# BruceCanovas/supersurfel_fusion

Measured on AMD Instinct MI355X. Metric: frames_per_sec, higher is better.
Workload: dtype f32; 1 GPU; 640x480 synthetic RGB-D orbit (seed 1234), map seeded with 1000000 supersurfels (~993223 live, ~86081 visible), reference rgbd_benchmark parameters, extract+ICP+fuse per frame; width=640, height=480, n_model=993223, n_visible=86081, superpixels=1200, icp_iter_max=10, icp_forced=False, seed_order=seeded, exchange=none, pipeline_depth=2, extract_batch=8

## Files before the change

### supersurfel_fusion_amd/csrc/lab/host_probes.inc

```

int ssf_dbg_last_icp_record(ssf_handle* h, int64_t* out29) {
    if (!h || !out29) return SSF_ERR_INVALID_ARG;
    for (int i = 0; i < 29; i++) out29[i] = h->h_icp_local[i];
    return SSF_OK;
}
int ssf_dbg_device_icp_records(ssf_handle* h, int64_t* out64) {
    if (!h || !out64) return SSF_ERR_INVALID_ARG;
    HCK(hipStreamSynchronize(h->stream));
    HCK(hipMemcpy(out64, h->d_icp, 64 * sizeof(int64_t), hipMemcpyDeviceToHost));
    return SSF_OK;
}
void ssf_dbg_stall_before_match_us(ssf_handle* h, long long us) { if (h) h->dbg_stall_before_match_us = us; }
long long ssf_dbg_assoc_replica_frames(ssf_handle* h) { return h ? h->n_assoc_replica_frames : -1; }
int ssf_dbg_host_times(ssf_handle* h, double* out8) {
    if (!h || !out8) return SSF_ERR_INVALID_ARG;
    for (int i = 0; i < 8; i++) { out8[i] = h->host_us[i]; h->host_us[i] = 0; }
    return SSF_OK;
}
double ssf_dbg_extract_only(ssf_handle* h, const void* const* rgb, const void* const* depth, int nlist, int n) {
    if (!h || !rgb || !depth || nlist <= 0 || !h->pending.empty()) return -1.0;
    int nsub = 0;
    double t0 = 0;
    for (int i = 0; i < n; i++) {
        if (i == n / 4) { for (auto& c : h->ctx) (void)hipStreamSynchronize(c.stream); (void)hipStreamSynchronize(h->stream); t0 = now_us(); }
// ... 46 lines not shown
    (void)hipStreamSynchronize(h->stream);
    float ms = 0.f; (void)hipEventElapsedTime(&ms, e0, e1);
    (void)hipEventDestroy(e0); (void)hipEventDestroy(e1);
    if (blocks2) {
        const int nb = (span + 255) / 256;
        std::vector<uint32_t> bc((size_t)std::max(nb, 1));
        if (nb > 0) (void)hipMemcpy(bc.data(), h->d_bc_oov, (size_t)nb * 4, hipMemcpyDeviceToHost);
        blocks2[0] = nb; blocks2[1] = 0;
        for (int i = 0; i < nb; i++) blocks2[1] += bc[i] != 0u;
    }
    return reps > 0 ? 1000.0 * ms / reps : 0.0;
}
int ssf_dbg_trace_fuse(ssf_handle* h, unsigned long long* out, int cap_wgs, int* arms4, int mode ) {
    if (!h || !h->have_frame || !h->cc || !out || !arms4) return -1;
    arms4[0] = (mode & 2) ? 0 : (h->S + 31) / 32; arms4[1] = (mode & 2) ? 0 : (h->S + 255) / 256; arms4[2] = (mode & 4) ? 0 : (h->n_visible + 255) / 256;
    long long b2[2];
    unsigned long long* d = nullptr;
    const size_t words = (size_t)3 * 65536;
    if (hipMalloc((void**)&d, words * 8) != hipSuccess) return -2;
    (void)hipMemset(d, 0, words * 8);
    set_fuse_trace(d);
    (void)ssf_dbg_time_fuse(h, 1, mode, b2);
    set_fuse_trace(nullptr);
    std::vector<unsigned long long> all(words);
    (void)hipMemcpy(all.data(), d, words * 8, hipMemcpyDeviceToHost);
    (void)hipFree(d);
    int n = 0;
    for (int i = 0; i < 65536; i++) if (all[3 * (size_t)i]) n = i + 1;
    arms4[3] = n - arms4[0] - arms4[1] - arms4[2];
    const int m = n < cap_wgs ? n : cap_wgs;
    std::memcpy(out, all.data(), (size_t)m * 24);
    return m;
}
int ssf_dbg_pass_stats_enable(int on) { set_pass_stats(on ? 1 : 0); return SSF_OK; }
int ssf_dbg_pass_stats(ssf_handle* h, uint32_t* out64) {
    if (!h || !h->active.ctx || !out64) return SSF_ERR_INVALID_ARG;
    HCK(hipStreamSynchronize(h->active.ctx->stream));
    HCK(hipMemcpy(out64, h->active.maps.epoch, 64 * sizeof(uint32_t), hipMemcpyDeviceToHost));
    return SSF_OK;
}
double ssf_dbg_time_pass(ssf_handle* h, int reps, int rgbd, int dbg, int nb) {
    if (!h || !h->active.ctx) return -1.0;
    ExtractCtx& c = *h->active.ctx;
    nb = std::max(1, std::min(nb, h->batch));
    hipEvent_t e0, e1; (void)hipEventCreate(&e0); (void)hipEventCreate(&e1);
    const int ox[4] = {0, 1, 0, 1}, oy[4] = {0, 1, 1, 0};
    for (int i = 0; i < 4; i++) launch_update_pass(h->stream, h->seg, c.maps, nb, 20 + i, ox[i & 3], oy[i & 3], rgbd != 0, dbg);
    (void)hipEventRecord(e0, h->stream);
    for (int i = 0; i < reps; i++) launch_update_pass(h->stream, h->seg, c.maps, nb, 24 + i, ox[i & 3], oy[i & 3], rgbd != 0, dbg);
    (void)hipEventRecord(e1, h->stream);
    (void)hipStreamSynchronize(h->stream);
    float ms = 0.f; (void)hipEventElapsedTime(&ms, e0, e1);
    (void)hipEventDestroy(e0); (void)hipEventDestroy(e1);
    return 1000.0 * ms / reps;
}
int ssf_dbg_trace_pass(ssf_handle* h, int rgbd, int nb, unsigned long long* out, int cap_wgs, int* grid3) {
    if (!h || !h->active.ctx || !out || !grid3) return -1;
    ExtractCtx& c = *h->active.ctx;
    nb = std::max(1, std::min(nb, h->batch));
    const int ox[4] = {0, 1, 0, 1}, oy[4] = {0, 1, 1, 0};
    grid3[0] = (h->cfg.width + 30 + 31) / 32; grid3[1] = (h->cfg.height + 31) / 32; grid3[2] = nb;
    const int n = grid3[0] * grid3[1] * grid3[2];
    unsigned long long* d = nullptr;
    if (hipMalloc((void**)&d, (size_t)n * 40) != hipSuccess) return -2;
    (void)hipMemset(d, 0, (size_t)n * 40);
    for (int i = 0; i < 4; i++) launch_update_pass(h->stream, h->seg, c.maps, nb, 20 + i, ox[i & 3], oy[i & 3], rgbd != 0, 0);
// ... 11 lines not shown
```

### supersurfel_fusion_amd/csrc/ssf_device.hpp

```cpp
#pragma once
#include <hip/hip_runtime.h>
#include <stdint.h>
#include <cstddef>
#include "ssf_math.hpp"
#include "ssf_mailbox.hpp"
#include "ssf_tile_geometry.hpp"
#include "../../include/ssf.h"
#include "../../include/ssf_input.h"
#include "../../include/ssf_dynamic.h"

#ifdef SSF_EXPERIMENTS
#include <stdlib.h>
static inline int ssf_env_int_(const char* name, int dflt) { const char* e = getenv(name); return e ? atoi(e) : dflt; }
#define SSF_ENV_INT(name, dflt) ssf_env_int_("SSF_" name, dflt)
#define SSF_ENV_SET(name) (getenv("SSF_" name) != nullptr)
#define SSF_ENV_STR(name) getenv("SSF_" name)
#define SSF_PROBE(dbg, bits) ((((dbg)) & (bits)) != 0)
#else
#define SSF_PROBE(dbg, bits) (false)
#define SSF_ENV_INT(name, dflt) (dflt)
#define SSF_ENV_SET(name) (false)
#define SSF_ENV_STR(name) ((const char*)nullptr)
#endif

// ... 152 lines not shown
SSF_HD int assoc_stride(int S) { return (S + 15) & ~15; }
SSF_HD size_t assoc_table_words(int S) { return (size_t)(1 + SSF_ASSOC_REPLICAS) * (size_t)assoc_stride(S); }
struct MatchArgs { float zmin, zmax; long long id_offset; unsigned long long* best; uint8_t* matched; int32_t* cand; int rstride; };
struct ClassifyArgs { Cam cam; const float* plane_depth; int delta_t; float conf_thresh, zmin, zmax; int assoc_rstride; };
struct ShardArgs { int rank, nranks, migrate; float tile; };
struct AssocTables { const unsigned long long* best; const uint8_t* matched; const int32_t* cand; int S; int rstride; };
int icp_variant_mode();
void launch_icp(hipStream_t st, const Cam& cam, SurfelSoA model, int n_visible, const uint2* pix2, const float4* fpack,
                Rt T, long long* replicas, unsigned int* ticket,
                long long* sums29, Mailbox* mb, unsigned long long seq, int dbg = -1, IcpGo* go = nullptr,
                unsigned long long go_seq = 0, const struct P2PView* pv = nullptr, int by_tile = 0, const MatchArgs* match = nullptr);
int icp_resident_max_wgs();
void launch_icp_resident(hipStream_t st, const Cam& cam, SurfelSoA model, int n_visible, const uint2* pix2, const float4* fpack, const Rt* T0,
                         long long* replicas, long long* sums29, Mailbox* mb, unsigned long long seq0, IcpGo* go, unsigned int go_base,
                         int last_idx, const MatchArgs* match);
void launch_bin_rows(hipStream_t st, const Cam& cam, SurfelSoA model, int n, Rt T, uint32_t* count, uint32_t* cursor, SurfelSoA out);
size_t bin_buffer_words(const Cam& cam, size_t capacity);
void launch_match(hipStream_t st, const Cam& cam, SurfelSoA model, int n_visible, const uint2* pix2, const float4* fpack,
                  Rt pose, float zmin, float zmax, long long id_offset,
                  unsigned long long* best, uint8_t* matched, int32_t* cand , int S,
                  const int32_t* orig = nullptr );
struct OovStore { SurfelSoA rows; uint8_t* live; int cap; };
#define PART_GROUP 16
#define PART_REPLICAS 8
struct PartitionWs { uint32_t* sup_vis; uint32_t* sup_oov; uint32_t* tot; uint32_t* ticket; uint32_t* other; int words; };
void launch_fuse(hipStream_t st, SurfelSoA model , SurfelSoA frame, Rt pose, int stamp, long long id_offset,
                 int n_visible, const AssocTables& at, int do_update, int capacity, const ShardArgs& sh, Counters* cnt, OovStore oov,
                 int span_upper, const ClassifyArgs& ca, uint8_t* state_vis, uint8_t* state_oov, uint32_t* bc_oov, const PartitionWs& ws,
                 int tail_in_move = 0 );
#ifdef SSF_EXPERIMENTS
void set_pass_stats(int on);
void set_pass_trace(unsigned long long* device_words );
void set_fuse_trace(unsigned long long* device_words );
#endif
struct MoveTotals { int from_tot, nv , head_old, tail_old ; };
void launch_pack_emigrants(hipStream_t st, SurfelSoA model, const AssocTables& at, long long id_offset, int n_visible,
                           const uint8_t* state_vis, int do_update, const ShardArgs& sh, int32_t* table);
void launch_migrate_in(hipStream_t st, SurfelSoA model, const int32_t* table, int S, int capacity, Counters* cnt, const ShardArgs& sh,
                       const ClassifyArgs& ca, Rt pose, int stamp, uint8_t* state_vis, const PartitionWs& ws);
void launch_rehome_split(hipStream_t st, SurfelSoA dense, int n, int n_visible, int rank, int nranks, float tile, uint32_t* bc, int* tot3,
                         SurfelSoA stay, int32_t* table, int table_rows);
void launch_rehome_unpack(hipStream_t st, const int32_t* table, int n, SurfelSoA dst, int base);
void launch_first_frame(hipStream_t st, SurfelSoA model, SurfelSoA frame, Rt pose, int S, int capacity, const ShardArgs& sh, Counters* cnt);
struct NextIcp {
    Cam cam; const uint2* pix2; const float4* fpack;
    Rt T;
    long long* replicas; unsigned int* ticket; long long* sums; Mailbox* mb; unsigned long long seq;
};
void launch_move_rows(hipStream_t st, SurfelSoA vis_src, SurfelSoA vis_dst, OovStore oov, int nv_upper, int span_upper,
                      const uint8_t* state_vis, const uint8_t* state_oov, const uint32_t* bc_oov, const PartitionWs& ws,
                      Counters* cnt , Mailbox* mb, unsigned long long cnt_seq, const NextIcp* next,
                      const struct P2PView* next_pv = nullptr, const MoveTotals* totals = nullptr);
void launch_oov_compact(hipStream_t st, OovStore src, OovStore dst, int span_upper, int new_head, uint32_t* bc_oov, Counters* cnt,
                        int set_span);
struct ModelView { SurfelSoA vis; OovStore oov; int n_visible, nbv, nvs, oov_head, oov_tail, nbo, nslots; };
void launch_align(hipStream_t st, const Cam& cam, const float* spos, const float* slab, const float* snrm, const float* sconf,
                  int n, SurfelSoA frame, const int32_t* label, const float* plane_depth, Rt T, long long* out40);
void launch_fern_codes(hipStream_t st, const uint8_t* rgb, const float* depth, int W, int H, const uint32_t* fpos,
                       const uint8_t* frgb, const float* fdepth, int n, uint8_t* codes);
#define SSF_P2P_MAX_RANKS 8
struct P2PView { unsigned char* peer[SSF_P2P_MAX_RANKS]; int me, nranks, S; unsigned long long seq, timeout_ticks; };
enum { P2P_FLAG_ASSOC = 0, P2P_FLAG_MIGR = 1 };
#define SSF_P2P_HEADER 8192
SSF_HD size_t p2p_slot(int par, int src) { return (size_t)(par * SSF_P2P_MAX_RANKS + src); }
SSF_HD size_t p2p_spad(int S) { return ((size_t)S + 63) & ~(size_t)63; }
SSF_HD size_t p2p_off_icp(int par, int src) { return p2p_slot(par, src) * 320; }
// ... 32 lines not shown
```

### supersurfel_fusion_amd/csrc/ssf_track_fuse.hip

```cpp
#include <stdlib.h>
#include <algorithm>
#include "ssf_rows.hpp"

namespace ssf {

#ifndef ICP_SLOTS
#define ICP_SLOTS 16
#endif
template <bool UNIFORM, typename Emit>
__device__ __forceinline__ void icp_row_terms_(const Cam& cam, const uint2* __restrict__ pix2, const float4* __restrict__ fpack,
                                               const M3& R, const V3& t, const V3& mpos, const V3& mlab, const V3& mnrm, int dbg, Emit emit,
                                               bool live = true) {
    const V3 ps = add(m3_mulv(R, mpos), t);
    if (SSF_PROBE(dbg, 1)) { if (ps.z > 1e30f) emit(28, 1ll); return; }
    const int u = pixel_round(ps.x * cam.fx / ps.z + cam.cx);
    const int v = pixel_round(ps.y * cam.fy / ps.z + cam.cy);
    bool ok = live && u >= 0 && u < cam.W && v >= 0 && v < cam.H;
    if (!UNIFORM && !ok) return;
    size_t q = ok ? (size_t)v * cam.W + u : 0;
    if (SSF_PROBE(dbg, 16)) q = (blockIdx.x * blockDim.x + threadIdx.x) & 0x7ffffu;
    const uint2 pl = pix2[q];
    const int tid = SSF_PROBE(dbg, 8) ? (int)(q & 1023) : (int)pl.x;
    const float zt = __uint_as_float(pl.y);
    float4 f0 = fpack[4 * tid], f1 = fpack[4 * tid + 1];
    asm volatile("" : "+v"(f0.y), "+v"(f1.x));
    ok = ok && (f0.x > 0.0f && zt >= 0.2f && zt <= 5.0f);
    if (!UNIFORM && !ok) return;
    const float dist_color = len3(sub(mlab, v3(f0.y, f0.z, f0.w)));
    const V3 pt = v3(zt * ((float)u - cam.cx) / cam.fx, zt * ((float)v - cam.cy) / cam.fy, zt);
    const V3 nt = v3(f1.x, f1.y, f1.z);
    const V3 ns = unit3(m3_mulv(R, mnrm));
    ok = ok && (dist_color < 20.0f && len3(sub(ps, pt)) < 0.1f && fabsf(dot3(nt, ns)) > 0.8f);
    if (!UNIFORM && !ok) return;
    const V3 d = sub(pt, ps), c1 = cross3(pt, ns), c2 = cross3(ps, nt);
    const float dn1 = dot3(d, ns), dn2 = dot3(d, nt);
    const float x1[6] = {c1.x, c1.y, c1.z, ns.x, ns.y, ns.z};
    const float x2[6] = {c2.x, c2.y, c2.z, nt.x, nt.y, nt.z};
    if (SSF_PROBE(dbg, 2)) { if (x1[0] * x2[0] > 1e30f) emit(0, 1ll); return; }
    const float m10 = (UNIFORM && !ok) ? 0.0f : 1024.0f, m14 = (UNIFORM && !ok) ? 0.0f : 16384.0f;
    float X1[6], X2[6];
#pragma unroll
    for (int i = 0; i < 6; i++) { X1[i] = UNIFORM && !ok ? 0.0f : x1[i] * m10; X2[i] = UNIFORM && !ok ? 0.0f : x2[i] * m10; }
    const float D1 = UNIFORM && !ok ? 0.0f : dn1 * m14, D2 = UNIFORM && !ok ? 0.0f : dn2 * m14;
    int k = 0;
#pragma unroll
    for (int i = 0; i < 6; i++)
#pragma unroll
        for (int j = i; j < 6; j++, k++) emit(k, (long long)fx32r(X1[i] * X1[j] + X2[i] * X2[j]));
#pragma unroll
    for (int i = 0; i < 6; i++) emit(21 + i, (long long)fx32r(D1 * X1[i] + D2 * X2[i]));
    emit(27, fx64((double)(UNIFORM && !ok ? 0.0f : dn2 * dn2), 17592186044416.0, 4611686018427387904.0));
    emit(28, (UNIFORM && !ok) ? 0ll : 1ll);
}
template <typename Emit>
__device__ __forceinline__ void icp_row_terms(const Cam& cam, const uint2* __restrict__ pix2, const float4* __restrict__ fpack,
                                              const M3& R, const V3& t, const V3& mpos, const V3& mlab, const V3& mnrm, int dbg, Emit emit) {
    icp_row_terms_<false>(cam, pix2, fpack, R, t, mpos, mlab, mnrm, dbg, emit);
}
__device__ __forceinline__ void icp_row(const Cam& cam, const uint2* __restrict__ pix2, const float4* __restrict__ fpack,
                                        const M3& R, const V3& t, const V3& mpos, const V3& mlab, const V3& mnrm,
                                        unsigned long long* red, int slot, int dbg) {
    icp_row_terms(cam, pix2, fpack, R, t, mpos, mlab, mnrm, dbg, [&](int k, long long v) { atomicAdd(&red[k * ICP_SLOTS + slot], (unsigned long long)v); });
}
__device__ __forceinline__ void icp_fold(unsigned long long* red, long long* __restrict__ replicas) {
    if (threadIdx.x < 29) {
        unsigned long long tot = 0;
#pragma unroll
        for (int sidx = 0; sidx < ICP_SLOTS; sidx++) tot += red[threadIdx.x * ICP_SLOTS + sidx];
        long long* rep = replicas + (size_t)(blockIdx.x % SSF_ICP_REPLICAS) * 32;
        if (tot != 0) atomic_add_done(reinterpret_cast<unsigned long long*>(&rep[threadIdx.x]), tot);
    }
    asm volatile("s_waitcnt vmcnt(0)" ::: "memory");
    __syncthreads();
}
template <bool P2P>
__device__ __forceinline__ void icp_publish(long long* __restrict__ replicas, long long* __restrict__ sums, Mailbox* mb,
                                            unsigned long long seq, const P2PView& pv, unsigned long long p2p_seq) {
    __shared__ long long part[8 * 32];
    const int field = threadIdx.x & 31, group = threadIdx.x >> 5;
    long long v = 0;
#pragma unroll
    for (int j = 0; j < (SSF_ICP_REPLICAS + 7) / 8; j++) {
        const int r = group + 8 * j;
        if (r < SSF_ICP_REPLICAS) {
            v += __hip_atomic_load(&replicas[r * 32 + field], __ATOMIC_RELAXED, __HIP_MEMORY_SCOPE_AGENT);
// ... 123 lines not shown
                                            float zmax, long long id_offset, unsigned long long* __restrict__ best,
                                            uint8_t* __restrict__ matched, bool wave_agg);
__device__ __forceinline__ void match_sorted_rows(const Cam& cam, const SurfelSoA& sorted, int n_visible, const uint2* __restrict__ pix2,
                                                  const float4* __restrict__ fpack, const Rt& pose, const MatchArgs& ma) {
    for (int j = (int)(xcd_block(blockIdx.x, gridDim.x) * blockDim.x + threadIdx.x); j < n_visible; j += gridDim.x * blockDim.x) {
        const float4* __restrict__ rec = reinterpret_cast<const float4*>(sorted.pos) + 3 * (size_t)j;
        float4 a = rec[0], b = rec[1], c = rec[2];
        asm volatile("" : "+v"(a.x), "+v"(b.x), "+v"(c.x));
        const int oid = __float_as_int(b.w);
        ma.cand[oid] = match_values(cam, a.w, v3(a.x, a.y, a.z), v3(c.x, c.y, c.z), v3(b.x, b.y, b.z), oid, pix2, fpack, pose, ma.zmin, ma.zmax, ma.id_offset, ma.best, ma.matched, true);
    }
}
__device__ __forceinline__ unsigned long long* assoc_bid_table(const MatchArgs& ma) {
    const unsigned int xcc = __builtin_amdgcn_s_getreg((3 << 11) | (0 << 6) | 20) & 7u;
    return ma.rstride ? ma.best + (size_t)(1u + xcc) * (size_t)ma.rstride : ma.best;
}
__device__ __forceinline__ unsigned long long assoc_best(const unsigned long long* __restrict__ best, int f, int rstride) {
    unsigned long long v = best[f];
    if (rstride) {
        unsigned long long r[SSF_ASSOC_REPLICAS];
#pragma unroll
        for (int x = 0; x < SSF_ASSOC_REPLICAS; x++) r[x] = best[(size_t)(1 + x) * (size_t)rstride + f];
#pragma unroll
        for (int x = 0; x < SSF_ASSOC_REPLICAS; x++) v = r[x] < v ? r[x] : v;
    }
    return v;
}
#define SSF_ICP_DBG_COUNTED 0x40000000
#ifndef SSF_ICP_GO_WAIT_TICKS
#define SSF_ICP_GO_WAIT_TICKS 25000000ull
#endif
#ifndef SSF_ICP_NUM_SGPR
#define SSF_ICP_NUM_SGPR 80
#endif
__device__ __forceinline__ int icp_wait_word(IcpGo* go, unsigned int want, unsigned int& w) {
    int ok = 0, told = 0;
    const unsigned int l = threadIdx.x;
    const unsigned int* gw = reinterpret_cast<const unsigned int*>(go);
    const unsigned int weight = icp_go_word_weight(l);
    w = 0u;
    const unsigned long long t0 = wall_clock64();
    for (unsigned int spin = 0; spin < (1u << 24); spin++) {
        w = l < 16u ? __hip_atomic_load(&gw[l], __ATOMIC_RELAXED, __HIP_MEMORY_SCOPE_SYSTEM) : 0u;
        const unsigned int flo = (unsigned int)__builtin_amdgcn_readlane((int)w, 12), fhi = (unsigned int)__builtin_amdgcn_readlane((int)w, 13);
        if (flo == want) {
            if (fhi & 0x80000000u) {
                if ((fhi & SSF_ICP_GO_CHECK_MASK) == icp_go_abort_check(want)) { told = 1; break; }
            } else {
                unsigned int sum = w * weight;
#pragma unroll
                for (int o = 1; o < 16; o <<= 1) sum += __shfl_xor(sum, o, 64);
                sum = (unsigned int)__builtin_amdgcn_readfirstlane((int)sum);
                if (((sum >> 2) & SSF_ICP_GO_CHECK_MASK) == (fhi & SSF_ICP_GO_CHECK_MASK)) {
                    ok = (fhi & 0x40000000u) ? 2 : 1; told = 1;
                    break;
                }
            }
        }
        if ((spin & 63u) == 63u && wall_clock64() - t0 > SSF_ICP_GO_WAIT_TICKS) break;
        __builtin_amdgcn_s_sleep(1);
    }
    if (!told && l == 0u) __hip_atomic_store(&go->flag, (unsigned long long)want | ((unsigned long long)icp_go_abort_check(want) << 32) | SSF_ICP_GO_ABORT, __ATOMIC_RELAXED, __HIP_MEMORY_SCOPE_SYSTEM);
    return ok;
}
template <bool P2P, int MODE>
__global__ __launch_bounds__(256) __attribute__((amdgpu_num_sgpr(SSF_ICP_NUM_SGPR))) void k_icp(Cam cam, SurfelSoA model, int n_visible,
// ... 465 lines not shown
        atomicAdd(&s_cls[(k >> 8) / PART_GROUP - g_first][st], 1u);
    }
    __syncthreads();
    if (threadIdx.x < 6) {
        const int seg = threadIdx.x / 3, st = threadIdx.x % 3;
        const uint32_t n = s_cls[seg][st];
        if (n) {
            atomicAdd(&ws.sup_vis[(g_first + seg) * 6 + 3 + st], n);
            atomic_add_done(&ws.tot[(chunk & (PART_REPLICAS - 1)) * 8 + 3 + st], n);
        }
    }
    if (chunk == nchunks - 1 && threadIdx.x == 0)
        atomic_store_done(&cnt->n_inserted, min(base_total + before + total, capacity) - base_total);
}
__device__ __forceinline__ Counters finalise_counters(Counters* cnt, Counters c, int shrink_by_removed, int keep_inserted = 0);
__device__ __forceinline__ void mailbox_counters(const Counters& c, Mailbox* mb, unsigned long long seq);
__device__ __forceinline__ Counters frame_counters(const Counters& c_in, const uint32_t* tot) {
    const int a0 = (int)tot[0], a1 = (int)tot[1], a2 = (int)tot[2], c0 = (int)tot[3], c1 = (int)tot[4], c2 = (int)tot[5];
    const int b0 = (int)tot[6], b2 = (int)tot[7], b1 = c_in.oov_live - b0 - b2;
    Counters c = c_in;
    c.n_model = c_in.n_model + c_in.n_inserted;
    c.n_state0 = a0 + b0 + c0; c.n_state1 = a1 + b1 + c1; c.n_state2 = a2 + b2 + c2;
    c.n_visible = a0 + b0 + c0; c.n_removed = (a2 + b2 + c2) - c_in.n_emigrated;
    c.mv_nv = c_in.n_visible; c.mv_a0 = a0; c.mv_b0 = b0; c.mv_nc = c_in.n_inserted;
    c.mv_head_old = c_in.oov_head; c.mv_tail_old = c_in.oov_tail; c.mv_head_new = c_in.oov_head - a1;
    c.oov_head = c_in.oov_head - a1; c.oov_tail = c_in.oov_tail + c1;
    c.oov_live = (c_in.oov_live - b0 - b2) + a1 + c1;
    return c;
}
#ifdef SSF_EXPERIMENTS
__device__ unsigned long long* g_fuse_trace = nullptr;
void set_fuse_trace(unsigned long long* p) { (void)hipMemcpyToSymbol(HIP_SYMBOL(g_fuse_trace), &p, sizeof(p)); }
#endif
__global__ __launch_bounds__(256) void k_update_insert(SurfelSoA M, SurfelSoA F, Rt pose, int stamp, long long id_offset,
                                                       int n_visible, const unsigned long long* __restrict__ best,
                                                       const uint8_t* __restrict__ matched, const int32_t* __restrict__ cand, int S,
                                                       int do_update, int capacity, int rank, int nranks, float tile, Counters* cnt,
                                                       int nupd, int nchunks, int nb_vis, int nb_oov, OovStore O, ClassifyArgs ca,
                                                       uint8_t* __restrict__ state_vis, uint8_t* __restrict__ state_oov,
                                                       uint32_t* __restrict__ bc_oov, PartitionWs ws, int migrate, int tail_in_move) {
    __builtin_amdgcn_s_setprio(3);
    __shared__ int wave_tot[16];
    __shared__ int hist[4][6];
    __shared__ int s_last;
    __shared__ uint32_t tot[8];
    const int b = blockIdx.x;
#ifdef SSF_EXPERIMENTS
    unsigned long long* const trace = g_fuse_trace;
    if (trace && threadIdx.x == 0) trace[3 * (size_t)b] = wall_clock64();
#endif
    if (b >= nupd + nchunks + nb_vis)
        classify_oov_block(ca.cam, O, pose, ca.plane_depth, stamp, ca.delta_t, ca.conf_thresh, ca.zmin, ca.zmax, state_oov, bc_oov,
                           ws, cnt, b - nupd - nchunks - nb_vis, nb_oov);
    else if (b >= nupd + nchunks) {
        const int vb = b - nupd - nchunks, i = vb * blockDim.x + threadIdx.x, wv = threadIdx.x >> 6;
        int cls = 7;
        if (i < n_visible) {
            int f = cand[i];
            float conf = M.conf[i]; int seen = M.stamps[2 * (size_t)i + 1]; V3 pos = ld3(M.pos, (size_t)i);
            asm volatile("" : "+v"(f), "+v"(conf), "+v"(seen), "+v"(pos.x));
            const bool rewritten = do_update && f >= 0 && (uint32_t)(assoc_best(best, f, ca.assoc_rstride) & 0xFFFFFFFFull) == (uint32_t)(id_offset + i);
            if (!rewritten) {
                cls = classify_values(ca.cam, conf, seen, pos, pose, ca.plane_depth, stamp, ca.delta_t, ca.conf_thresh, ca.zmin, ca.zmax);
                if (cls == 2) M.conf[i] = -1.0f;
                state_vis[i] = (uint8_t)cls;
            }
        }
// ... 42 lines not shown
        c_in.n_inserted = __hip_atomic_load(&cnt->n_inserted, __ATOMIC_RELAXED, __HIP_MEMORY_SCOPE_AGENT);
        c_in.n_updated = __hip_atomic_load(&cnt->n_updated, __ATOMIC_RELAXED, __HIP_MEMORY_SCOPE_AGENT);
        c_in.n_emigrated = __hip_atomic_load(&cnt->n_emigrated, __ATOMIC_RELAXED, __HIP_MEMORY_SCOPE_AGENT);
        cnt[1] = finalise_counters(cnt, frame_counters(c_in, tot), 1);
    }
}

__global__ __launch_bounds__(1024) void k_first_frame(SurfelSoA M, SurfelSoA F, Rt pose, int S, int capacity, int rank,
                                                      int nranks, float tile, Counters* cnt) {
    __shared__ int wave_tot[16];
    int running = 0;
    for (int c0 = 0; c0 < S; c0 += 1024) {
        const int f = c0 + threadIdx.x;
        const bool flag = (f < S) && shard_owner(F, f, pose, nranks, tile) == rank;
        int total;
        const int r = block_rank_1024(flag, wave_tot, total);
        const int k = running + r;
        if (flag && k < capacity) {
            st3(M.pos, k, ld3(F.pos, f)); st3(M.col, k, ld3(F.col, f)); st3(M.lab, k, ld3(F.lab, f));
            M.stamps[2 * k] = F.stamps[2 * f]; M.stamps[2 * k + 1] = F.stamps[2 * f + 1];
            st3(M.r0, k, ld3(F.r0, f)); st3(M.r1, k, ld3(F.r1, f)); st3(M.r2, k, ld3(F.r2, f));
            st6(M.shape, k, ld6(F.shape, f));
            M.dims[2 * k] = F.dims[2 * f]; M.dims[2 * k + 1] = F.dims[2 * f + 1];
            M.conf[k] = F.conf[f];
        }
        running += total;
    }
    if (threadIdx.x == 0) {
        const int n = min(running, capacity);
        cnt->n_model = n; cnt->n_visible = n; cnt->n_inserted = 0; cnt->n_removed = 0;
    }
}

__device__ __forceinline__ void copy_row_keep(const SurfelSoA& A, size_t i, const SurfelSoA& B, size_t j, V3& pos, V3& lab, V3& nrm) {
    const RowRegs r = load_row(A, i);
    pos = r.pos; lab = r.lab; nrm = r.r2;
    store_row(B, j, r);
}
template <bool ICP, bool P2P>
__global__ __launch_bounds__(256) void k_move_rows(SurfelSoA V, SurfelSoA Vn, OovStore O, const uint8_t* __restrict__ state_vis,
                                                   const uint8_t* __restrict__ state_oov,
                                                   const uint32_t* __restrict__ bc_oov, PartitionWs ws,
                                                   Counters* cnt, int nb_vis, NextIcp nx, Mailbox* mb,
                                                   unsigned long long cnt_seq, P2PView pv, MoveTotals mt) {
    __builtin_amdgcn_s_setprio(3);
    if (blockIdx.x == 0 && threadIdx.x == 255) {
        Counters c;
        if (mt.from_tot) {
            uint32_t tot[8];
#pragma unroll
            for (int k = 0; k < 8; k++) {
                uint32_t v = 0;
#pragma unroll
                for (int r = 0; r < PART_REPLICAS; r++) v += __builtin_nontemporal_load(&ws.tot[r * 8 + k]);
                tot[k] = v;
            }
            const Counters c_in = *cnt;
            c = finalise_counters(cnt, frame_counters(c_in, tot), 1, 1);
            cnt[1] = c;
        } else {
            int w[sizeof(Counters) / sizeof(int)];
            const int* src = reinterpret_cast<const int*>(&cnt[1]);
#pragma unroll
            for (int i = 0; i < (int)(sizeof(Counters) / sizeof(int)); i++) w[i] = __builtin_nontemporal_load(&src[i]);
            __builtin_memcpy(&c, w, sizeof(c));
        }
        mailbox_counters(c, mb, cnt_seq);
    }
    if (mt.from_tot && blockIdx.x == 0 && threadIdx.x >= 64 && threadIdx.x < 255)
        for (int i = threadIdx.x - 64; i < ws.words; i += 191) ws.other[i] = 0u;
    if ((int)blockIdx.x >= nb_vis && bc_oov[blockIdx.x - nb_vis] == 0u) return;
    __shared__ uint32_t s_tot[8];
    if (mt.from_tot && threadIdx.x < 8) {
        uint32_t v = 0;
#pragma unroll
        for (int r = 0; r < PART_REPLICAS; r++) v += ws.tot[r * 8 + threadIdx.x];
        s_tot[threadIdx.x] = v;
    }
    const int mv_nv = mt.from_tot ? mt.nv : cnt->mv_nv, mv_nc = mt.from_tot ? cnt->n_inserted : cnt->mv_nc;
    const int mv_head_old = mt.from_tot ? mt.head_old : cnt->mv_head_old, mv_tail_old = mt.from_tot ? mt.tail_old : cnt->mv_tail_old;
    auto mv_a0 = [&]() -> int { return mt.from_tot ? (int)s_tot[0] : cnt->mv_a0; };
    auto mv_b0 = [&]() -> int { return mt.from_tot ? (int)s_tot[6] : cnt->mv_b0; };
    auto mv_head_new = [&]() -> int { return mt.from_tot ? mt.head_old - (int)s_tot[1] : cnt->mv_head_new; };
    auto new_n_visible = [&]() -> int { return mt.from_tot ? (int)(s_tot[0] + s_tot[6] + s_tot[3]) : cnt->n_visible; };
    __shared__ int hist[4][6];
    __shared__ uint32_t base[6];
    __shared__ unsigned long long red[ICP ? 29 * ICP_SLOTS : 1];
    if (ICP) for (int i = threadIdx.x; i < 29 * ICP_SLOTS; i += blockDim.x) red[i] = 0ull;
    if (threadIdx.x < 6) base[threadIdx.x] = 0u;
    const int wv = threadIdx.x >> 6;
    int cls = 7, in_wave = 0;
    bool keep = false;
    V3 pos, lab, nrm;
    if ((int)blockIdx.x < nb_vis) {
        const int nv = mv_nv, n_rows = nv + mv_nc;
        const int i = blockIdx.x * blockDim.x + threadIdx.x;
        RowRegs row;
        if (i < n_rows) {
            int st = (int)state_vis[i];
            row = load_row(V, i);
            asm volatile("" : "+v"(st), "+v"(row.pos.x));
            cls = (i < nv ? 0 : 3) + st;
        }
        const int g0 = (int)(blockIdx.x / PART_GROUP), ng = 6 * g0;
        const int row0 = g0 * PART_GROUP * 256, n16 = 16 * ((int)blockIdx.x - g0 * PART_GROUP);
        __syncthreads();
        for (int w = threadIdx.x; w < ng; w += blockDim.x) {
            const uint32_t v = ws.sup_vis[w];
            if (v) atomicAdd(&base[w % 6], v);
        }
        uint32_t pa0 = 0, pa1 = 0, pc0 = 0, pc1 = 0;
        for (int q = threadIdx.x; q < n16; q += blockDim.x) {
            const int r0 = row0 + 16 * q;
            if (r0 < n_rows) {
                const uint4 sv = *reinterpret_cast<const uint4*>(state_vis + r0);
                const uint32_t wd[4] = {sv.x, sv.y, sv.z, sv.w};
                uint32_t a0 = 0, a1 = 0, c0 = 0, c1 = 0;
#pragma unroll
                for (int j = 0; j < 16; j++) {
                    const int rr = r0 + j;
                    const uint32_t stt = (wd[j >> 2] >> (8 * (j & 3))) & 0xFFu;
                    const bool in = rr < n_rows, old = rr < nv;
                    a0 += (in && old && stt == 0u) ? 1u : 0u; a1 += (in && old && stt == 1u) ? 1u : 0u;
                    c0 += (in && !old && stt == 0u) ? 1u : 0u; c1 += (in && !old && stt == 1u) ? 1u : 0u;
                }
                pa0 += a0; pa1 += a1; pc0 += c0; pc1 += c1;
            }
        }
#pragma unroll
        for (int o = 32; o > 0; o >>= 1) {
            pa0 += __shfl_xor(pa0, o, 64); pa1 += __shfl_xor(pa1, o, 64); pc0 += __shfl_xor(pc0, o, 64); pc1 += __shfl_xor(pc1, o, 64);
        }
        if (lane() == 0) {
            if (pa0) atomicAdd(&base[0], pa0);
            if (pa1) atomicAdd(&base[1], pa1);
            if (pc0) atomicAdd(&base[3], pc0);
            if (pc1) atomicAdd(&base[4], pc1);
        }
#pragma unroll
        for (int c = 0; c < 6; c++) {
            const unsigned long long mask = __ballot(cls == c);
            if (cls == c) in_wave = __popcll(mask & ((1ull << lane()) - 1ull));
            if (lane() == 0) hist[wv][c] = __popcll(mask);
        }
        __syncthreads();
        if (cls == 0 || cls == 1 || cls == 3 || cls == 4) {
            int before = 0;
            for (int w = 0; w < wv; w++) before += hist[w][cls];
            const size_t r = (size_t)base[cls] + before + in_wave;
            if (cls == 0 || cls == 3) {
                const size_t j = cls == 0 ? r : (size_t)mv_a0() + mv_b0() + r;
                store_row(Vn, j, row);
                if (ICP) { pos = row.pos; lab = row.lab; nrm = row.r2; keep = true; }
            } else {
                const size_t j = (cls == 1 ? (size_t)mv_head_new() : (size_t)mv_tail_old) + r;
                store_row(O.rows, j, row);
                O.live[j] = 1;
            }
        }
    } else {
        const int ob = blockIdx.x - nb_vis;
        const long long phys = (long long)mv_head_old + (long long)ob * blockDim.x + threadIdx.x;
        if (phys < mv_tail_old) {
            int lv = (int)O.live[phys], st = (int)state_oov[phys];
            asm volatile("" : "+v"(lv), "+v"(st));
            if (lv) cls = st;
        }
        const unsigned long long mask = __ballot(cls == 0);
        if (cls == 0) in_wave = __popcll(mask & ((1ull << lane()) - 1ull));
        if (lane() == 0) hist[wv][0] = __popcll(mask);
        if (__syncthreads_count(cls == 0)) {
            const int g0 = ob / PART_GROUP, nw = g0 + (ob - g0 * PART_GROUP);
            for (int w = threadIdx.x; w < nw; w += blockDim.x) {
                const uint32_t v = w < g0 ? ws.sup_oov[w] : (bc_oov[g0 * PART_GROUP + (w - g0)] & 0xFFFFu);
                if (v) atomicAdd(&base[0], v);
            }
            __syncthreads();
        }
        if (cls == 0) {
            int before = 0;
            for (int w = 0; w < wv; w++) before += hist[w][0];
            const size_t j = (size_t)mv_a0() + base[0] + before + in_wave;
            if (ICP) { copy_row_keep(O.rows, (size_t)phys, Vn, j, pos, lab, nrm); keep = true; }
            else copy_row(O.rows, (size_t)phys, Vn, j);
        }
        if (cls == 0 || cls == 2) O.live[phys] = 0;
    }
    if (ICP) {
        if (keep) icp_row(nx.cam, nx.pix2, nx.fpack, nx.T.R, nx.T.t, pos, lab, nrm, red, lane() & (ICP_SLOTS - 1), 0);
        const int nkeep = __syncthreads_count(keep);
        if (P2P && new_n_visible() == 0) {
            if (blockIdx.x == 0) icp_publish<true>(nx.replicas, nx.sums, nx.mb, nx.seq, pv, pv.seq);
            return;
        }
        const bool vis = (int)blockIdx.x < nb_vis;
        const int nbr = (mv_nv + mv_nc + 255) / 256;
        if (vis ? (int)blockIdx.x >= nbr : nkeep == 0) return;
        __shared__ int s_last;
        icp_fold(red, nx.replicas);
        if (threadIdx.x == 0) {
            SSF_ARRIVE_RELEASE();
            unsigned int rows = (unsigned int)nkeep;
            bool report = true;
            if (vis) {
                const unsigned int g = blockIdx.x & 63u, in_group = ((unsigned int)nbr - g + 63u) / 64u;
                unsigned long long* gw = reinterpret_cast<unsigned long long*>(nx.ticket + 128) + g;
                const unsigned long long before = __hip_atomic_fetch_add(gw, ((unsigned long long)rows << 32) | 1ull, __ATOMIC_RELAXED,
                                                                         __HIP_MEMORY_SCOPE_AGENT);
                report = (unsigned int)(before & 0xFFFFFFFFull) == in_group - 1;
                if (report) {
                    rows += (unsigned int)(before >> 32);
                    __hip_atomic_store(gw, 0ull, __ATOMIC_RELAXED, __HIP_MEMORY_SCOPE_AGENT);
                }
            }
            int last = 0;
            if (report) {
                const unsigned int total = (unsigned int)new_n_visible();
                const unsigned int before = rows ? __hip_atomic_fetch_add(&nx.ticket[65], rows, __ATOMIC_RELAXED, __HIP_MEMORY_SCOPE_AGENT) : 0u;
                last = rows != 0u && before + rows == total;
                if (last) __hip_atomic_store(&nx.ticket[65], 0u, __ATOMIC_RELAXED, __HIP_MEMORY_SCOPE_AGENT);
            }
            if (last) SSF_ARRIVE_ACQUIRE();
            s_last = last;
        }
        __syncthreads();
        if (s_last) icp_publish<P2P>(nx.replicas, nx.sums, nx.mb, nx.seq, pv, pv.seq);
    }
}

__global__ __launch_bounds__(256) void k_pack_emigrants(SurfelSoA M, const unsigned long long* __restrict__ best,
                                                        const uint8_t* __restrict__ matched, long long id_offset, int n_visible,
                                                        const uint8_t* __restrict__ state_vis, int S, int do_update, int nranks,
                                                        float tile, int32_t* __restrict__ table) {
    const int f = blockIdx.x * blockDim.x + threadIdx.x;
    if (f >= S) return;
    int32_t w[SSF_MIGRANT_WORDS];
#pragma unroll
    for (int i = 0; i < SSF_MIGRANT_WORDS; i++) w[i] = 0;
    const unsigned long long bk = assoc_best(best, f, 0);
    if (do_update && matched[f] && bk != SSF_NO_MATCH) {
        const long long local = (long long)(uint32_t)(bk & 0xFFFFFFFFull) - id_offset;
        if (local >= 0 && local < n_visible) {
            const size_t m = (size_t)local;
            const float conf = M.conf[m];
            if (state_vis[m] == 2 && conf > 0.0f) {
                const RowRegs r = load_row(M, m);
                w[0] = tile_owner(r.pos, nranks, tile) + 1;
                migrant_pack(r, w);
            }
        }
    }
    int32_t* o = table + (size_t)SSF_MIGRANT_WORDS * f;
#pragma unroll
    for (int i = 0; i < SSF_MIGRANT_WORDS; i++) o[i] = w[i];
}
__global__ __launch_bounds__(1024) void k_migrate_in(SurfelSoA M, const int32_t* __restrict__ table, int S, int rank, int capacity,
                                                     Counters* cnt, ClassifyArgs ca, Rt pose, int stamp,
                                                     uint8_t* __restrict__ state_vis, PartitionWs ws) {
    __shared__ int wave_tot[16];
    __shared__ int s_in[4];
// ... 163 lines not shown
```

Baseline: 12420 frames/s.

## Overlap ICP gathers with partition scans in move-rows kernel and early-exit idle blocks

```diff
diff --git a/supersurfel_fusion_amd/csrc/lab/host_probes.inc b/supersurfel_fusion_amd/csrc/lab/host_probes.inc
--- a/supersurfel_fusion_amd/csrc/lab/host_probes.inc
+++ b/supersurfel_fusion_amd/csrc/lab/host_probes.inc
@@ -102,6 +102,32 @@
     std::memcpy(out, all.data(), (size_t)m * 24);
     return m;
 }
+static unsigned long long* g_move_trace_words = nullptr;
+int ssf_dbg_move_trace(int on) {
+    const size_t bytes = (size_t)8 * 65536 * sizeof(unsigned long long);
+    if (on && !g_move_trace_words) {
+        if (hipMalloc((void**)&g_move_trace_words, bytes) != hipSuccess) return SSF_ERR_INVALID_ARG;
+        (void)hipMemset(g_move_trace_words, 0, bytes);
+        set_move_trace(g_move_trace_words);
+    } else if (!on && g_move_trace_words) {
+        (void)hipDeviceSynchronize();
+        set_move_trace(nullptr);
+        (void)hipFree(g_move_trace_words);
+        g_move_trace_words = nullptr;
+    }
+    return SSF_OK;
+}
+int ssf_dbg_move_trace_read(ssf_handle* h, unsigned long long* out, int cap_wgs) {
+    if (!h || !out || !g_move_trace_words) return -1;
+    (void)hipStreamSynchronize(h->stream);
+    std::vector<unsigned long long> all((size_t)8 * 65536);
+    (void)hipMemcpy(all.data(), g_move_trace_words, all.size() * 8, hipMemcpyDeviceToHost);
+    int n = 0;
+    for (int i = 0; i < 65536; i++) if (all[8 * (size_t)i]) n = i + 1;
+    const int m = n < cap_wgs ? n : cap_wgs;
+    std::memcpy(out, all.data(), (size_t)m * 64);
+    return m;
+}
 int ssf_dbg_pass_stats_enable(int on) { set_pass_stats(on ? 1 : 0); return SSF_OK; }
 int ssf_dbg_pass_stats(ssf_handle* h, uint32_t* out64) {
     if (!h || !h->active.ctx || !out64) return SSF_ERR_INVALID_ARG;
diff --git a/supersurfel_fusion_amd/csrc/ssf_device.hpp b/supersurfel_fusion_amd/csrc/ssf_device.hpp
--- a/supersurfel_fusion_amd/csrc/ssf_device.hpp
+++ b/supersurfel_fusion_amd/csrc/ssf_device.hpp
@@ -208,6 +208,7 @@
 void set_pass_stats(int on);
 void set_pass_trace(unsigned long long* device_words );
 void set_fuse_trace(unsigned long long* device_words );
+void set_move_trace(unsigned long long* device_words );
 #endif
 struct MoveTotals { int from_tot, nv , head_old, tail_old ; };
 void launch_pack_emigrants(hipStream_t st, SurfelSoA model, const AssocTables& at, long long id_offset, int n_visible,
diff --git a/supersurfel_fusion_amd/csrc/ssf_track_fuse.hip b/supersurfel_fusion_amd/csrc/ssf_track_fuse.hip
--- a/supersurfel_fusion_amd/csrc/ssf_track_fuse.hip
+++ b/supersurfel_fusion_amd/csrc/ssf_track_fuse.hip
@@ -7,23 +7,22 @@
 #ifndef ICP_SLOTS
 #define ICP_SLOTS 16
 #endif
+struct IcpLook { V3 ps; int u, v; bool ok; size_t q; };
+__device__ __forceinline__ IcpLook icp_look(const Cam& cam, const V3& ps, bool live) {
+    IcpLook l;
+    l.ps = ps;
+    l.u = pixel_round(ps.x * cam.fx / ps.z + cam.cx);
+    l.v = pixel_round(ps.y * cam.fy / ps.z + cam.cy);
+    l.ok = live && l.u >= 0 && l.u < cam.W && l.v >= 0 && l.v < cam.H;
+    l.q = l.ok ? (size_t)l.v * cam.W + l.u : 0;
+    return l;
+}
 template <bool UNIFORM, typename Emit>
-__device__ __forceinline__ void icp_row_terms_(const Cam& cam, const uint2* __restrict__ pix2, const float4* __restrict__ fpack,
-                                               const M3& R, const V3& t, const V3& mpos, const V3& mlab, const V3& mnrm, int dbg, Emit emit,
-                                               bool live = true) {
-    const V3 ps = add(m3_mulv(R, mpos), t);
-    if (SSF_PROBE(dbg, 1)) { if (ps.z > 1e30f) emit(28, 1ll); return; }
-    const int u = pixel_round(ps.x * cam.fx / ps.z + cam.cx);
-    const int v = pixel_round(ps.y * cam.fy / ps.z + cam.cy);
-    bool ok = live && u >= 0 && u < cam.W && v >= 0 && v < cam.H;
-    if (!UNIFORM && !ok) return;
-    size_t q = ok ? (size_t)v * cam.W + u : 0;
-    if (SSF_PROBE(dbg, 16)) q = (blockIdx.x * blockDim.x + threadIdx.x) & 0x7ffffu;
-    const uint2 pl = pix2[q];
-    const int tid = SSF_PROBE(dbg, 8) ? (int)(q & 1023) : (int)pl.x;
-    const float zt = __uint_as_float(pl.y);
-    float4 f0 = fpack[4 * tid], f1 = fpack[4 * tid + 1];
-    asm volatile("" : "+v"(f0.y), "+v"(f1.x));
+__device__ __forceinline__ void icp_terms_gathered(const Cam& cam, const M3& R, const IcpLook& l, float zt, const float4& f0, const float4& f1,
+                                                   const V3& mlab, const V3& mnrm, int dbg, Emit emit) {
+    const V3& ps = l.ps;
+    const int u = l.u, v = l.v;
+    bool ok = l.ok;
     ok = ok && (f0.x > 0.0f && zt >= 0.2f && zt <= 5.0f);
     if (!UNIFORM && !ok) return;
     const float dist_color = len3(sub(mlab, v3(f0.y, f0.z, f0.w)));
@@ -51,6 +50,23 @@
     for (int i = 0; i < 6; i++) emit(21 + i, (long long)fx32r(D1 * X1[i] + D2 * X2[i]));
     emit(27, fx64((double)(UNIFORM && !ok ? 0.0f : dn2 * dn2), 17592186044416.0, 4611686018427387904.0));
     emit(28, (UNIFORM && !ok) ? 0ll : 1ll);
+}
+template <bool UNIFORM, typename Emit>
+__device__ __forceinline__ void icp_row_terms_(const Cam& cam, const uint2* __restrict__ pix2, const float4* __restrict__ fpack,
+                                               const M3& R, const V3& t, const V3& mpos, const V3& mlab, const V3& mnrm, int dbg, Emit emit,
+                                               bool live = true) {
+    const V3 ps = add(m3_mulv(R, mpos), t);
+    if (SSF_PROBE(dbg, 1)) { if (ps.z > 1e30f) emit(28, 1ll); return; }
+    const IcpLook l = icp_look(cam, ps, live);
+    if (!UNIFORM && !l.ok) return;
+    size_t q = l.q;
+    if (SSF_PROBE(dbg, 16)) q = (blockIdx.x * blockDim.x + threadIdx.x) & 0x7ffffu;
+    const uint2 pl = pix2[q];
+    const int tid = SSF_PROBE(dbg, 8) ? (int)(q & 1023) : (int)pl.x;
+    const float zt = __uint_as_float(pl.y);
+    float4 f0 = fpack[4 * tid], f1 = fpack[4 * tid + 1];
+    asm volatile("" : "+v"(f0.y), "+v"(f1.x));
+    icp_terms_gathered<UNIFORM>(cam, R, l, zt, f0, f1, mlab, mnrm, dbg, emit);
 }
 template <typename Emit>
 __device__ __forceinline__ void icp_row_terms(const Cam& cam, const uint2* __restrict__ pix2, const float4* __restrict__ fpack,
@@ -240,6 +256,12 @@
 #endif
 #ifndef SSF_ICP_NUM_SGPR
 #define SSF_ICP_NUM_SGPR 80
+#endif
+#ifndef SSF_FUSE_NUM_SGPR
+#define SSF_FUSE_NUM_SGPR 96
+#endif
+#ifndef SSF_MOVE_NUM_SGPR
+#define SSF_MOVE_NUM_SGPR 80
 #endif
 __device__ __forceinline__ int icp_wait_word(IcpGo* go, unsigned int want, unsigned int& w) {
     int ok = 0, told = 0;
@@ -771,7 +793,7 @@
 __device__ unsigned long long* g_fuse_trace = nullptr;
 void set_fuse_trace(unsigned long long* p) { (void)hipMemcpyToSymbol(HIP_SYMBOL(g_fuse_trace), &p, sizeof(p)); }
 #endif
-__global__ __launch_bounds__(256) void k_update_insert(SurfelSoA M, SurfelSoA F, Rt pose, int stamp, long long id_offset,
+__global__ __launch_bounds__(256) __attribute__((amdgpu_num_sgpr(SSF_FUSE_NUM_SGPR))) void k_update_insert(SurfelSoA M, SurfelSoA F, Rt pose, int stamp, long long id_offset,
                                                        int n_visible, const unsigned long long* __restrict__ best,
                                                        const uint8_t* __restrict__ matched, const int32_t* __restrict__ cand, int S,
                                                        int do_update, int capacity, int rank, int nranks, float tile, Counters* cnt,
@@ -880,18 +902,26 @@
     }
 }
 
-__device__ __forceinline__ void copy_row_keep(const SurfelSoA& A, size_t i, const SurfelSoA& B, size_t j, V3& pos, V3& lab, V3& nrm) {
-    const RowRegs r = load_row(A, i);
-    pos = r.pos; lab = r.lab; nrm = r.r2;
-    store_row(B, j, r);
-}
+#ifdef SSF_EXPERIMENTS
+__device__ unsigned long long* g_move_trace = nullptr;
+void set_move_trace(unsigned long long* p) { (void)hipMemcpyToSymbol(HIP_SYMBOL(g_move_trace), &p, sizeof(p)); }
+#define MOVE_TICK(k) do { if (trace && threadIdx.x == 0) trace[k] = wall_clock64(); } while (0)
+#define MOVE_KIND(k) do { if (trace && threadIdx.x == 0) trace[7] = (unsigned long long)(k) | (ICP ? 0x100ull : 0ull); } while (0)
+#else
+#define MOVE_TICK(k) do { } while (0)
+#define MOVE_KIND(k) do { } while (0)
+#endif
 template <bool ICP, bool P2P>
-__global__ __launch_bounds__(256) void k_move_rows(SurfelSoA V, SurfelSoA Vn, OovStore O, const uint8_t* __restrict__ state_vis,
+__global__ __launch_bounds__(256, 6) __attribute__((amdgpu_num_sgpr(SSF_MOVE_NUM_SGPR))) void k_move_rows(SurfelSoA V, SurfelSoA Vn, OovStore O, const uint8_t* __restrict__ state_vis,
                                                    const uint8_t* __restrict__ state_oov,
                                                    const uint32_t* __restrict__ bc_oov, PartitionWs ws,
                                                    Counters* cnt, int nb_vis, NextIcp nx, Mailbox* mb,
                                                    unsigned long long cnt_seq, P2PView pv, MoveTotals mt) {
     __builtin_amdgcn_s_setprio(3);
+#ifdef SSF_EXPERIMENTS
+    unsigned long long* const trace = (g_move_trace && blockIdx.x < 65536u) ? g_move_trace + 8 * (size_t)blockIdx.x : nullptr;
+    if (trace && threadIdx.x < 8) trace[threadIdx.x] = threadIdx.x == 0 ? wall_clock64() : 0ull;
+#endif
     if (blockIdx.x == 0 && threadIdx.x == 255) {
         Counters c;
         if (mt.from_tot) {
@@ -917,7 +947,23 @@
     }
     if (mt.from_tot && blockIdx.x == 0 && threadIdx.x >= 64 && threadIdx.x < 255)
         for (int i = threadIdx.x - 64; i < ws.words; i += 191) ws.other[i] = 0u;
-    if ((int)blockIdx.x >= nb_vis && bc_oov[blockIdx.x - nb_vis] == 0u) return;
+    const bool vis = (int)blockIdx.x < nb_vis;
+    const uint32_t bc = vis ? 0u : bc_oov[blockIdx.x - nb_vis];
+    if (!vis && bc == 0u) { MOVE_KIND(4); MOVE_TICK(6); return; }
+    const int mv_nv = mt.from_tot ? mt.nv : cnt->mv_nv, mv_nc = mt.from_tot ? cnt->n_inserted : cnt->mv_nc;
+    const int mv_head_old = mt.from_tot ? mt.head_old : cnt->mv_head_old, mv_tail_old = mt.from_tot ? mt.tail_old : cnt->mv_tail_old;
+    const int nbr = (mv_nv + mv_nc + 255) / 256;
+    if (vis && (int)blockIdx.x >= nbr && !(P2P && blockIdx.x == 0)) { MOVE_KIND(1 + 16); MOVE_TICK(6); return; }
+    if (!vis && (bc & 0xFFFFu) == 0u) {
+        const long long phys = (long long)mv_head_old + (long long)(blockIdx.x - nb_vis) * blockDim.x + threadIdx.x;
+        if (phys < mv_tail_old) {
+            int lv = (int)O.live[phys], st = (int)state_oov[phys];
+            asm volatile("" : "+v"(lv), "+v"(st));
+            if (lv && st == 2) O.live[phys] = 0;
+        }
+        MOVE_KIND(3); MOVE_TICK(6);
+        return;
+    }
     __shared__ uint32_t s_tot[8];
     if (mt.from_tot && threadIdx.x < 8) {
         uint32_t v = 0;
@@ -925,12 +971,11 @@
         for (int r = 0; r < PART_REPLICAS; r++) v += ws.tot[r * 8 + threadIdx.x];
         s_tot[threadIdx.x] = v;
     }
-    const int mv_nv = mt.from_tot ? mt.nv : cnt->mv_nv, mv_nc = mt.from_tot ? cnt->n_inserted : cnt->mv_nc;
-    const int mv_head_old = mt.from_tot ? mt.head_old : cnt->mv_head_old, mv_tail_old = mt.from_tot ? mt.tail_old : cnt->mv_tail_old;
-    auto mv_a0 = [&]() -> int { return mt.from_tot ? (int)s_tot[0] : cnt->mv_a0; };
-    auto mv_b0 = [&]() -> int { return mt.from_tot ? (int)s_tot[6] : cnt->mv_b0; };
-    auto mv_head_new = [&]() -> int { return mt.from_tot ? mt.head_old - (int)s_tot[1] : cnt->mv_head_new; };
-    auto new_n_visible = [&]() -> int { return mt.from_tot ? (int)(s_tot[0] + s_tot[6] + s_tot[3]) : cnt->n_visible; };
+    const int c_a0 = cnt->mv_a0, c_b0 = cnt->mv_b0, c_head_new = cnt->mv_head_new, c_n_visible = cnt->n_visible;
+    auto mv_a0 = [&]() -> int { const int t = (int)s_tot[0]; return mt.from_tot ? t : c_a0; };
+    auto mv_b0 = [&]() -> int { const int t = (int)s_tot[6]; return mt.from_tot ? t : c_b0; };
+    auto mv_head_new = [&]() -> int { const int t = mt.head_old - (int)s_tot[1]; return mt.from_tot ? t : c_head_new; };
+    auto new_n_visible = [&]() -> int { const int t = (int)(s_tot[0] + s_tot[6] + s_tot[3]); return mt.from_tot ? t : c_n_visible; };
     __shared__ int hist[4][6];
     __shared__ uint32_t base[6];
     __shared__ unsigned long long red[ICP ? 29 * ICP_SLOTS : 1];
@@ -939,51 +984,72 @@
     const int wv = threadIdx.x >> 6;
     int cls = 7, in_wave = 0;
     bool keep = false;
-    V3 pos, lab, nrm;
-    if ((int)blockIdx.x < nb_vis) {
+    IcpLook lk{};
+    uint2 pl = make_uint2(0u, 0u);
+    float4 f0 = make_float4(0.f, 0.f, 0.f, 0.f), f1 = f0;
+    V3 lab = v3(0.f, 0.f, 0.f), nrm = lab;
+    auto icp_look_row = [&](const RowRegs& r) { lab = r.lab; nrm = r.r2; lk = icp_look(nx.cam, add(m3_mulv(nx.T.R, r.pos), nx.T.t), true); };
+    auto icp_first_gather = [&]() { pl = nx.pix2[lk.q]; };
+    auto icp_second_gather = [&]() {
+        asm volatile("" : "+v"(pl.x), "+v"(pl.y));
+        const int tid = lk.ok ? (int)pl.x : 0;
+        f0 = nx.fpack[4 * tid]; f1 = nx.fpack[4 * tid + 1];
+    };
+    auto icp_terms = [&]() {
+        asm volatile("" : "+v"(f0.x), "+v"(f0.y), "+v"(f1.x));
+        if (lk.ok) {
+            const int slot = lane() & (ICP_SLOTS - 1);
+            icp_terms_gathered<false>(nx.cam, nx.T.R, lk, __uint_as_float(pl.y), f0, f1, lab, nrm, 0,
+                                      [&](int k, long long v) { atomicAdd(&red[k * ICP_SLOTS + slot], (unsigned long long)v); });
+        }
+    };
+    if (vis) {
         const int nv = mv_nv, n_rows = nv + mv_nc;
         const int i = blockIdx.x * blockDim.x + threadIdx.x;
         RowRegs row;
         if (i < n_rows) {
             int st = (int)state_vis[i];
             row = load_row(V, i);
-            asm volatile("" : "+v"(st), "+v"(row.pos.x));
+            asm volatile("" : "+v"(st), "+v"(row.pos.x), "+v"(row.pos.y), "+v"(row.pos.z));
             cls = (i < nv ? 0 : 3) + st;
         }
+        MOVE_KIND(1); MOVE_TICK(1);
+        keep = cls == 0 || cls == 3;
+        if (ICP && keep) icp_look_row(row);
+        if (ICP) icp_first_gather();
         const int g0 = (int)(blockIdx.x / PART_GROUP), ng = 6 * g0;
         const int row0 = g0 * PART_GROUP * 256, n16 = 16 * ((int)blockIdx.x - g0 * PART_GROUP);
+        static_assert(16 * (PART_GROUP - 1) <= 256, "one 16-byte state load per thread covers the earlier blocks of a group");
+        const int r0 = row0 + 16 * (int)threadIdx.x;
+        const bool have_sup = (int)threadIdx.x < ng, have_sv = (int)threadIdx.x < n16 && r0 < n_rows;
+        uint32_t sup = ws.sup_vis[have_sup ? threadIdx.x : 0];
+        uint4 sv = *reinterpret_cast<const uint4*>(state_vis + (have_sv ? r0 : 0));
+        if (ICP) icp_second_gather();
+        asm volatile("" : "+v"(sup), "+v"(sv.x), "+v"(sv.y), "+v"(sv.z), "+v"(sv.w));
+        uint32_t pa = 0u, pc = 0u;
+        if (have_sv) {
+            const uint32_t wd[4] = {sv.x, sv.y, sv.z, sv.w};
+#pragma unroll
+            for (int j = 0; j < 16; j++) {
+                const int rr = r0 + j;
+                const uint32_t stt = (wd[j >> 2] >> (8 * (j & 3))) & 0xFFu;
+                const uint32_t one = stt == 0u ? 1u : (stt == 1u ? 0x10000u : 0u);
+                if (rr < nv) pa += one; else if (rr < n_rows) pc += one;
+            }
+        }
         __syncthreads();
-        for (int w = threadIdx.x; w < ng; w += blockDim.x) {
+        if (have_sup && sup) atomicAdd(&base[threadIdx.x % 6], sup);
+        for (int w = threadIdx.x + blockDim.x; w < ng; w += blockDim.x) {
             const uint32_t v = ws.sup_vis[w];
             if (v) atomicAdd(&base[w % 6], v);
         }
-        uint32_t pa0 = 0, pa1 = 0, pc0 = 0, pc1 = 0;
-        for (int q = threadIdx.x; q < n16; q += blockDim.x) {
-            const int r0 = row0 + 16 * q;
-            if (r0 < n_rows) {
-                const uint4 sv = *reinterpret_cast<const uint4*>(state_vis + r0);
-                const uint32_t wd[4] = {sv.x, sv.y, sv.z, sv.w};
-                uint32_t a0 = 0, a1 = 0, c0 = 0, c1 = 0;
-#pragma unroll
-                for (int j = 0; j < 16; j++) {
-                    const int rr = r0 + j;
-                    const uint32_t stt = (wd[j >> 2] >> (8 * (j & 3))) & 0xFFu;
-                    const bool in = rr < n_rows, old = rr < nv;
-                    a0 += (in && old && stt == 0u) ? 1u : 0u; a1 += (in && old && stt == 1u) ? 1u : 0u;
-                    c0 += (in && !old && stt == 0u) ? 1u : 0u; c1 += (in && !old && stt == 1u) ? 1u : 0u;
-                }
-                pa0 += a0; pa1 += a1; pc0 += c0; pc1 += c1;
-            }
-        }
-#pragma unroll
-        for (int o = 32; o > 0; o >>= 1) {
-            pa0 += __shfl_xor(pa0, o, 64); pa1 += __shfl_xor(pa1, o, 64); pc0 += __shfl_xor(pc0, o, 64); pc1 += __shfl_xor(pc1, o, 64);
-        }
+#pragma unroll
+        for (int o = 32; o > 0; o >>= 1) { pa += __shfl_xor(pa, o, 64); pc += __shfl_xor(pc, o, 64); }
         if (lane() == 0) {
-            if (pa0) atomicAdd(&base[0], pa0);
-            if (pa1) atomicAdd(&base[1], pa1);
-            if (pc0) atomicAdd(&base[3], pc0);
-            if (pc1) atomicAdd(&base[4], pc1);
+            if (pa & 0xFFFFu) atomicAdd(&base[0], pa & 0xFFFFu);
+            if (pa >> 16) atomicAdd(&base[1], pa >> 16);
+            if (pc & 0xFFFFu) atomicAdd(&base[3], pc & 0xFFFFu);
+            if (pc >> 16) atomicAdd(&base[4], pc >> 16);
         }
 #pragma unroll
         for (int c = 0; c < 6; c++) {
@@ -992,20 +1058,22 @@
             if (lane() == 0) hist[wv][c] = __popcll(mask);
         }
         __syncthreads();
+        MOVE_TICK(2);
+        if (ICP) icp_terms();
         if (cls == 0 || cls == 1 || cls == 3 || cls == 4) {
             int before = 0;
             for (int w = 0; w < wv; w++) before += hist[w][cls];
             const size_t r = (size_t)base[cls] + before + in_wave;
-            if (cls == 0 || cls == 3) {
+            if (keep) {
                 const size_t j = cls == 0 ? r : (size_t)mv_a0() + mv_b0() + r;
                 store_row(Vn, j, row);
-                if (ICP) { pos = row.pos; lab = row.lab; nrm = row.r2; keep = true; }
             } else {
                 const size_t j = (cls == 1 ? (size_t)mv_head_new() : (size_t)mv_tail_old) + r;
                 store_row(O.rows, j, row);
                 O.live[j] = 1;
             }
         }
+        MOVE_TICK(3);
     } else {
         const int ob = blockIdx.x - nb_vis;
         const long long phys = (long long)mv_head_old + (long long)ob * blockDim.x + threadIdx.x;
@@ -1014,38 +1082,54 @@
             asm volatile("" : "+v"(lv), "+v"(st));
             if (lv) cls = st;
         }
-        const unsigned long long mask = __ballot(cls == 0);
-        if (cls == 0) in_wave = __popcll(mask & ((1ull << lane()) - 1ull));
+        MOVE_KIND(2); MOVE_TICK(1);
+        keep = cls == 0;
+        RowRegs row;
+        if (keep) {
+            row = load_row(O.rows, (size_t)phys);
+            if (ICP) {
+                asm volatile("" : "+v"(row.pos.x), "+v"(row.pos.y), "+v"(row.pos.z));
+                icp_look_row(row);
+            }
+        }
+        if (ICP) icp_first_gather();
+        const unsigned long long mask = __ballot(keep);
+        if (keep) in_wave = __popcll(mask & ((1ull << lane()) - 1ull));
         if (lane() == 0) hist[wv][0] = __popcll(mask);
-        if (__syncthreads_count(cls == 0)) {
-            const int g0 = ob / PART_GROUP, nw = g0 + (ob - g0 * PART_GROUP);
-            for (int w = threadIdx.x; w < nw; w += blockDim.x) {
-                const uint32_t v = w < g0 ? ws.sup_oov[w] : (bc_oov[g0 * PART_GROUP + (w - g0)] & 0xFFFFu);
-                if (v) atomicAdd(&base[0], v);
-            }
-            __syncthreads();
-        }
-        if (cls == 0) {
+        const int g0 = ob / PART_GROUP, nw = g0 + (ob - g0 * PART_GROUP);
+        auto returning_before = [&](int w) -> uint32_t { return *(w < g0 ? &ws.sup_oov[w] : &bc_oov[g0 * PART_GROUP + (w - g0)]) & 0xFFFFu; };
+        const bool have_sup = (int)threadIdx.x < nw;
+        uint32_t sup = returning_before(have_sup ? (int)threadIdx.x : 0);
+        if (ICP) icp_second_gather();
+        asm volatile("" : "+v"(sup));
+        __syncthreads();
+        if (have_sup && sup) atomicAdd(&base[0], sup);
+        for (int w = threadIdx.x + blockDim.x; w < nw; w += blockDim.x) {
+            const uint32_t v = returning_before(w);
+            if (v) atomicAdd(&base[0], v);
+        }
+        __syncthreads();
+        MOVE_TICK(2);
+        if (ICP) icp_terms();
+        if (keep) {
             int before = 0;
             for (int w = 0; w < wv; w++) before += hist[w][0];
-            const size_t j = (size_t)mv_a0() + base[0] + before + in_wave;
-            if (ICP) { copy_row_keep(O.rows, (size_t)phys, Vn, j, pos, lab, nrm); keep = true; }
-            else copy_row(O.rows, (size_t)phys, Vn, j);
+            store_row(Vn, (size_t)mv_a0() + base[0] + before + in_wave, row);
         }
         if (cls == 0 || cls == 2) O.live[phys] = 0;
+        MOVE_TICK(3);
     }
     if (ICP) {
-        if (keep) icp_row(nx.cam, nx.pix2, nx.fpack, nx.T.R, nx.T.t, pos, lab, nrm, red, lane() & (ICP_SLOTS - 1), 0);
         const int nkeep = __syncthreads_count(keep);
+        MOVE_TICK(4);
         if (P2P && new_n_visible() == 0) {
             if (blockIdx.x == 0) icp_publish<true>(nx.replicas, nx.sums, nx.mb, nx.seq, pv, pv.seq);
             return;
         }
-        const bool vis = (int)blockIdx.x < nb_vis;
-        const int nbr = (mv_nv + mv_nc + 255) / 256;
-        if (vis ? (int)blockIdx.x >= nbr : nkeep == 0) return;
+        if (vis ? (int)blockIdx.x >= nbr : nkeep == 0) { MOVE_TICK(6); return; }
         __shared__ int s_last;
         icp_fold(red, nx.replicas);
+        MOVE_TICK(5);
         if (threadIdx.x == 0) {
             SSF_ARRIVE_RELEASE();
             unsigned int rows = (unsigned int)nkeep;
@@ -1074,6 +1158,7 @@
         __syncthreads();
         if (s_last) icp_publish<P2P>(nx.replicas, nx.sums, nx.mb, nx.seq, pv, pv.seq);
     }
+    MOVE_TICK(6);
 }
 
 __global__ __launch_bounds__(256) void k_pack_emigrants(SurfelSoA M, const unsigned long long* __restrict__ best,
```

Result: faster. 12700 frames/s, median of 6 (+2.3%).
